# MasterBin-IIAU/Unicorn

Measured on NVIDIA H100. Metric: frames/sec, higher is better.
Workload: dtype bf16

## Files before the change

### include/unicorn_b200.h

```cpp
#ifndef UNICORN_B200_H_
#define UNICORN_B200_H_
#include <stdint.h>

#ifdef __cplusplus
extern "C" {
#endif

#if defined(__GNUC__)
#define UC_API __attribute__((visibility("default")))
#else
#define UC_API
#endif

#define UC_OK 0
#define UC_EINVAL (-1)
#define UC_EDRIVER (-2)
#define UC_ENODEV (-3)

#define UC_BF16 0
#define UC_F32 1
#define UC_F16 2

#define UC_ACT_NONE 0
#define UC_ACT_RELU 1
#define UC_ACT_GELU 2
#define UC_ACT_SILU 3
#define UC_ACT_SIGMOID 4

UC_API const char* uc_last_error(void);
UC_API int uc_version(void);
UC_API int uc_check_device(void);

typedef struct UcConv2d {
  const void* x;
  int x_dtype;
  int B, H, W, Cin, ldx;
  const void* w;
  int Cout, KH, KW, stride, pad;
  const float* bias;
  int act;
  const float* gamma;
  const void* res;
  int ldres;
  void* y;
  int ldy;
  int y_dtype;
  int block_n;
  void* gn_stats;
  int gn_groups;
  const void* row_stats;
  const float* col_s;
  float row_eps;
  int act_after_res;
} UcConv2d;
UC_API int uc_conv2d(const UcConv2d* d, void* stream);

UC_API int uc_stem_ln(const void* img, int img_is_u8_hwc, const float* w48, const float* bias, const float* lnw, const float* lnb,
                      void* out_bf16, int B, int H, int W, int C0, float eps, void* stream);

UC_API int uc_resnet_stem(const void* img, int img_is_u8_hwc, const void* w_f16, const float* bias, void* out_bf16, int B, int H, int W,
                          void* stream);

UC_API int uc_dwconv7_ln(const void* x_bf16, const float* w49, const float* bias, const float* lnw, const float* lnb,
                         void* y_bf16, int B, int H, int W, int C, float eps, void* stream);

UC_API int uc_dwconv7(const void* x_bf16, const float* w49, const float* bias, void* y_bf16, int B, int H, int W, int C,
                      void* ln_stats, int* work_counter, void* stream);

UC_API int uc_dwconv7_mma(const void* x_bf16, const void* qtab, void* y_bf16, int B, int H, int W, int C, int* work_counter, void* stream);

UC_API int uc_convnext_mlp_supported(int C);
UC_API int uc_convnext_mlp(const void* t_bf16, const void* w1f_bf16, const float* c1, const void* w2_bf16, const float* b2, const float* gamma,
                           void* x_bf16, int M, int C, float ln_eps, void* stream);

UC_API int uc_layernorm(const void* x, int ldx, const void* res, int ldres, const float* w, const float* b, void* y,
                        int ldy, long M, int C, float eps, int dtype, void* stream);

UC_API int uc_groupnorm_apply(const void* x, int ldx, const void* stats, const float* w, const float* b, void* y,
                              int ldy, int B, long HW, int C, int G, float eps, int act, const float* prior,
                              const float* beta, const void* add2, int ldadd2, void* y2, int ldy2, void* stream);
UC_API int uc_groupnorm_apply_gather(const void* x, int ldx, int n_src, const void* stats, const float* w, const float* b, void* y,
                                     int ldy, int B, int n_plain, const int* src_of, long HW, int C, int G, float eps, int act,
                                     const float* prior, const float* beta, void* stream);

UC_API int uc_copy_upsample(const void* src, int lds, void* dst, int ldd, int B, int Hs, int Ws, int C, int up, void* stream);
UC_API int uc_pixel_shuffle2(const void* in, int ldi, void* out, int ldo, int B, int H, int W, int Co, void* stream);
UC_API int uc_bilinear_f32(const float* src, float* dst, int P, int Hs, int Ws, int Hd, int Wd, float scale_h,
                           float scale_w, void* stream);
UC_API int uc_letterbox_u8(const uint8_t* src_hwc, int Hs, int Ws, uint8_t* dst_hwc, int Hd, int Wd, int rh, int rw,
                           int swap_rb, int pad, void* stream);
UC_API int uc_letterbox_nv12(const uint8_t* y, const uint8_t* uv, int ld, int Hs, int Ws, uint8_t* dst_hwc, int Hd, int Wd, int rh,
                             int rw, int pad, void* stream);
UC_API int uc_add(const void* a, int lda, const void* b, int ldb, void* y, int ldy, long M, int C, int dtype, void* stream);
UC_API int uc_copy_rows_if(const int* flag_dev, int invert, const void* src, long src_ld_bytes, void* dst, long dst_ld_bytes, long rows,
                           int row_bytes, void* stream);
UC_API int uc_copy_rows_if_batched(const int* flag_dev, const int* gate_dev, int invert, const void* src, long src_ld_bytes, long src_bs_bytes,
                                   void* dst, long dst_ld_bytes, long dst_bs_bytes, long rows, int row_bytes, int B, void* stream);
UC_API int uc_nchw_f32_to_nhwc(const float* src, void* dst, int ldd, int B, int C, long HW, int dtype, void* stream);
UC_API int uc_nhwc_to_nchw_f32(const void* src, int lds, float* dst, int B, int C, long HW, int dtype, void* stream);

UC_API int uc_msda_forward_f32(const float* value, const int64_t* spatial_shapes, const int64_t* level_start_index,
                               const float* sampling_loc, const float* attn_weight, int B, int S, int M, int D, int L,
                               int Lq, int P, float* out, void* stream);
UC_API int uc_msda_fused_bf16(const void* value, const float* offlog, int ld_offlog, void* out, const int* level_hw,
                              int L, int M, int P, void* stream);
UC_API int uc_msda_fused_bf16_batched(const void* value, const float* offlog, int ld_offlog, void* out, const int* level_hw,
                                      int L, int M, int P, int B, void* stream);

UC_API int uc_corr_propagate(const void* embed_ref, int ld_ref, int n_ref, const void* embed_cur, int ld_cur, int n_cur,
                             int C, int dtype, const float* values, int ldv, int n_obj, float* out, int ldo, void* stream);
UC_API int uc_corr_propagate_batched(const void* embed_ref, int ld_ref, long bs_ref, int n_ref, const void* embed_cur, int ld_cur,
                                     long bs_cur, int n_cur, int C, int dtype, const float* values, int ldv, long bs_values, int n_obj,
                                     float* out, int ldo, long bs_out, int B, void* stream);

UC_API int uc_head_decode(const float* const* regobj, const float* const* cls, const int* hw, const int* strides,
                          int ld_ro, int ld_cls, int ncls, float* out, void* stream);
UC_API int uc_head_decode_batched(const float* const* regobj, const float* const* cls, const int* hw, const int* strides,
                                  int ld_ro, int ld_cls, const long* bs_ro, const long* bs_cls, int ncls, int B, float* out,
                                  void* stream);

UC_API long uc_postprocess_workspace_bytes(int max_anchors);
UC_API int uc_postprocess(const float* pred, int A, int ncls, float conf_thre, float nms_thre, int max_keep, void* workspace,
                          long workspace_bytes, float* out_dets, int* out_count, int* out_anchor, void* stream);
UC_API long uc_postprocess_workspace_bytes_batched(int max_anchors, int B);
UC_API int uc_postprocess_batched(const float* pred, int A, int ncls, float conf_thre, float nms_thre, int max_keep, int B,
                                  void* workspace, long workspace_bytes, float* out_dets, int* out_count, int* out_anchor, void* stream);

#define UC_POST_CLASS_AGNOSTIC 1
UC_API int uc_postprocess_batched_ex(const float* pred, int A, int ncls, float conf_thre, float nms_thre, int max_keep, int B, int flags,
                                     void* workspace, long workspace_bytes, float* out_dets, int* out_count, int* out_anchor, void* stream);
UC_API int uc_det_candidates_batched(const float* const* regobj, const float* const* cls, const int* hw, const int* strides, int ld_ro,
                                     int ld_cls, const long* bs_ro, const long* bs_cls, int ncls, int B, float conf_thre, void* workspace,
                                     long workspace_bytes, void* stream);
UC_API int uc_postprocess_nms_batched(int A, float nms_thre, int max_keep, int B, int flags, void* workspace, long workspace_bytes,
                                      float* out_dets, int* out_count, int* out_anchor, void* stream);

UC_API int uc_sample_embed(const void* embed, int ld, int h, int w, int C, int dtype, const float* boxes, int ldb,
                           const int* count_dev, int n_max, float stride, float* out, void* stream);
UC_API int uc_sample_embed_batched(const void* embed, int ld, long bs_embed, int h, int w, int C, int dtype, const float* boxes, int ldb,
                                   long bs_boxes, const int* count_dev, int n_max, float stride, float* out, long bs_out, int B, void* stream);
UC_API int uc_bisoftmax(const float* det_embeds, const float* memo_embeds, int N, int M, int C, const float* det_labels,
                        const float* memo_labels, float* workspace, float* scores, void* stream);
UC_API int uc_qd_assign(const float* scores, int N, int M, const long long* memo_ids, const float* det_scores, int ld_det, float match_thr,
                        float obj_thr, float nms_conf_thr, long long* ids_out, uint8_t* taken_ws, void* stream);
UC_API int uc_box_iou(const float* a, int lda, int N, const float* b, int ldb, int M, float* out, int plus_one, void* stream);

UC_API int uc_aligned_bilinear_add(const void* src, int lds, int hs, int ws, void* dst, int ldd, int C, int factor, void* stream);
UC_API int uc_aligned_bilinear_add_batched(const void* src, int lds, long bs_src, int hs, int ws, void* dst, int ldd, long bs_dst, int C,
                                           int factor, int B, void* stream);
UC_API int uc_dynamic_masks(const float* mask_feats, const float* up_masks, int h, int w, int up_rate, int d_rate,
                            const float* const* dyn_levels, int ld_dyn, const int* level_hw, const int* level_strides,
                            const float* level_soi, const int* anchors_dev, const int* count_dev, int n_max, float* scratch,
                            float* out_masks, void* stream);
UC_API int uc_dynamic_masks_batched(const float* mask_feats, const float* up_masks, int S, int h, int w, int up_rate, int d_rate,
                                    const float* const* dyn_levels, int ld_dyn, const long* bs_dyn, const int* level_hw,
                                    const int* level_strides, const float* level_soi, const int* anchors_dev, long bs_anchors,
                                    const int* count_dev, const int* image_of, int B, int n_max, float* scratch, float* out_masks,
                                    void* stream);

typedef struct UcVosObject {
  const float* mask;
  const uint8_t* init_mask;
  int id;
} UcVosObject;
UC_API int uc_vos_aggregate(const UcVosObject* objs, int n, int Hin, int Win, int H, int W, float r, float* soft_out,
                            uint8_t* seg_out, void* stream);

#define UC_VOS_MAX_VIDEOS UC_MOTS_MAX_IMAGES
typedef struct UcVosVideo {
  const UcVosObject* objs;
  int n;
  int H, W;
  float r;
  float* soft_out;
  uint8_t* seg_out;
} UcVosVideo;
UC_API int uc_vos_aggregate_batched(const UcVosVideo* videos, int B, int Hin, int Win, void* stream);

UC_API long uc_mots_encode_workspace_bytes(int k_max, int H, int W);
UC_API int uc_mots_encode(const float* masks, int n_max, int Hin, int Win, const int* order, const uint8_t* emit, int k, float thr,
                          double r, int H, int W, void* workspace, long workspace_bytes, char* chars, long capacity,
                          long long* offsets, void* stream);

#define UC_MOTS_MAX_IMAGES 64
UC_API int uc_mots_encode_batched(const float* masks, long bs_masks, int n_max, int Hin, int Win, int B, const int* k, const int* H,
                                  const int* W, const double* r, const int* order, const uint8_t* emit, float thr, void* workspace,
                                  long workspace_bytes, char* chars, long capacity, long long* offsets, void* stream);

UC_API int uc_inst_encode_batched(const float* maps, long bs_maps, int n_max, int hs, int ws, int d_rate, int B, const int* count_dev,
                                  int row0, const int* H, const int* W, const double* r, float thr, void* workspace, long workspace_bytes,
                                  uint8_t* emit, char* chars, long capacity, long long* offsets, void* stream);

#define UC_BDD_BAD_CHARS 1
#define UC_BDD_BAD_RUNS 2
#define UC_BDD_BAD_INDEX 4
UC_API long uc_bdd_bitmask_workspace_bytes(int B, const int* k, const int* H, const int* W, long n_chars);
UC_API int uc_bdd_bitmask_batched(int B, const int* k, const int* H, const int* W, const long* out_offsets, const char* chars, long n_chars,
                                  const long long* offsets, const uint32_t* colors, const int* ranks, void* workspace, long workspace_bytes,
                                  uint8_t* out, long out_bytes, int* status, void* stream);

#ifdef __cplusplus
}
#endif
#endif
```

### unicorn_b200/csrc/dwconv_mma.cu

```cuda
#include "uc_ptx.cuh"
#include "uc_common.h"
#include "../../include/unicorn_b200.h"
#include <algorithm>

namespace uc {

constexpr int kMmTW = 16, kMmTH = 16, kMmCH = 32;
constexpr int kMmHW = kMmTW + 8, kMmHH = kMmTH + 6;
constexpr int kMmPixBytes = kMmCH * 2;
constexpr int kMmStageBytes = kMmHH * kMmHW * kMmPixBytes;
constexpr int kMmPlaneBytes = kMmHH * kMmHW * 2;
constexpr int kMmPlanarBytes = kMmCH * kMmPlaneBytes;
constexpr int kMmPairBytes = kMmCH * 7 * 8 * 4;
constexpr int kMmQBytes = kMmPairBytes + kMmCH * 4;
constexpr int kMmSmem = kMmStageBytes + kMmPlanarBytes + kMmQBytes + 128 + 128;
constexpr int kMmWarps = 4, kMmCtasPerSm = 3;

struct alignas(64) DwMmaParams {
  CUtensorMap tmX;
  const uint8_t* qtab;
  uint16_t* y;
  int* work_counter;
  int H, W, C, B, tiles_w, tiles_h, n_items;
};

__device__ __forceinline__ int mm_plane(int c) { return (c & 7) * 4 + (c >> 3); }

__device__ __forceinline__ void bulk_load_1d(void* smem, const void* gmem, uint32_t bytes, uint64_t* bar) {
  asm volatile("cp.async.bulk.shared::cluster.global.mbarrier::complete_tx::bytes [%0], [%1], %2, [%3];" ::"r"(smem_u32(smem)), "l"(gmem),
               "r"(bytes), "r"(smem_u32(bar))
               : "memory");
}

struct DwFrag {
  uint32_t a[2][6];
  uint32_t q[2];
};

__global__ void __launch_bounds__(kMmWarps * 32, kMmCtasPerSm) dwconv7_mma_kernel(const __grid_constant__ DwMmaParams p) {
  constexpr int CPW = kMmCH / kMmWarps;
  extern __shared__ uint8_t dsm_raw[];
  uint8_t* stage = dsm_raw + ((128u - (smem_u32(dsm_raw) & 127u)) & 127u);
  uint8_t* planar = stage + kMmStageBytes;
  uint8_t* qs = planar + kMmPlanarBytes;
  uint64_t* bar = reinterpret_cast<uint64_t*>(qs + kMmQBytes);
  volatile int* s_info = reinterpret_cast<volatile int*>(bar + 2);
  const int lane = threadIdx.x & 31, warp = threadIdx.x >> 5;
  const int g = lane >> 2, t = lane & 3;
  if (threadIdx.x == 0) {
    prefetch_tmap(&p.tmX);
    mbar_init(&bar[0], 1);
    mbar_init(&bar[1], 1);
    fence_barrier_init();
  }
  __syncthreads();
  pdl_wait();
  pdl_launch_dependents();
  const int tiles_img = p.tiles_w * p.tiles_h, tiles_chunk = tiles_img * p.B;
  int static_next = blockIdx.x;
  auto fetch = [&]() {
    if (p.work_counter) return atomicAdd(p.work_counter, 1);
    const int item = static_next;
    static_next += gridDim.x;
    return item;
  };
  auto issue = [&](int slot, int item) {
    volatile int* info = s_info + slot * 4;
    if (item >= p.n_items) {
      info[0] = -1;
      mbar_arrive(&bar[0]);
      return;
    }
    const int chunk = item / tiles_chunk, tt0 = item - chunk * tiles_chunk;
    const int b = tt0 / tiles_img, tt = tt0 - b * tiles_img;
    const int oh0 = (tt / p.tiles_w) * kMmTH, ow0 = (tt % p.tiles_w) * kMmTW;
    info[0] = chunk; info[1] = b; info[2] = oh0; info[3] = ow0;
    mbar_arrive_expect_tx(&bar[0], kMmStageBytes);
    tma_load_4d(stage, &p.tmX, &bar[0], chunk * kMmCH, ow0 - 4, oh0 - 3, b);
  };
  int pending = 0;
  if (threadIdx.x == 0) {
    issue(0, fetch());
    pending = fetch();
  }
  const int fc = warp * CPW;
  const uint32_t planar_w = smem_u32(planar) + mm_plane(fc) * kMmPlaneBytes;
  const uint32_t lm4 = planar_w + static_cast<uint32_t>((((lane & 7) + ((lane >> 3) & 1) * 8) * kMmHW + (lane >> 4) * 8) * 2);
  const uint32_t lm2 = planar_w + static_cast<uint32_t>(((lane & 15) * kMmHW + 16) * 2);
  const int d = 2 * t - g - 1;
  const bool first = d >= -1;
  const uint32_t q_lane = smem_u32(qs) + static_cast<uint32_t>((fc * 7 * 8 + (first ? d + 1 : d + 9)) * 4);
  const float* bias_s = reinterpret_cast<const float*>(qs + kMmPairBytes) + fc;
  const int tq = lane & 3, tsw = (lane >> 2) & 1;
  const uint32_t sel_lo = tsw ? 0x1054u : 0x5410u, sel_hi = tsw ? 0x3276u : 0x7632u;
  auto load_frag = [&](int s, DwFrag& f) {
    const int kh = s % 7;
#pragma unroll
    for (int j = 0; j < 2; ++j) {
      const int c = (s / 7) * 2 + j;
      const uint32_t off = static_cast<uint32_t>(c * 4 * kMmPlaneBytes + kh * (kMmHW * 2));
      asm volatile("ldmatrix.sync.aligned.m8n8.x4.shared.b16 {%0,%1,%2,%3}, [%4];"
                   : "=r"(f.a[j][0]), "=r"(f.a[j][1]), "=r"(f.a[j][2]), "=r"(f.a[j][3]) : "r"(lm4 + off));
      asm volatile("ldmatrix.sync.aligned.m8n8.x2.shared.b16 {%0,%1}, [%2];" : "=r"(f.a[j][4]), "=r"(f.a[j][5]) : "r"(lm2 + off));
      asm volatile("ld.shared.b32 %0, [%1];" : "=r"(f.q[j]) : "r"(q_lane + static_cast<uint32_t>((c * 7 + kh) * 32)));
    }
  };
  int prev_chunk = -1;
  uint32_t q_phase = 0;
  for (int it = 0;; ++it) {
    mbar_wait(&bar[0], it & 1);
    const int chunk = s_info[(it & 1) * 4 + 0];
    if (chunk < 0) break;
    const int b = s_info[(it & 1) * 4 + 1], oh0 = s_info[(it & 1) * 4 + 2], ow0 = s_info[(it & 1) * 4 + 3];
    const int c0 = chunk * kMmCH + fc;
    const bool new_chunk = chunk != prev_chunk;
    prev_chunk = chunk;
    if (new_chunk && threadIdx.x == 0) {
      mbar_arrive_expect_tx(&bar[1], kMmQBytes);
      bulk_load_1d(qs, p.qtab + static_cast<size_t>(chunk) * kMmQBytes, kMmQBytes, &bar[1]);
    }
    {
      const uint4* st = reinterpret_cast<const uint4*>(stage);
#pragma unroll 3
      for (int pp = warp * 8 + (lane >> 2); pp < kMmHH * kMmHW / 2; pp += kMmWarps * 8) {
        const uint4 va = st[(2 * pp + tsw) * 4 + tq];
        const uint4 vb = st[(2 * pp + (tsw ^ 1)) * 4 + tq];
        const uint32_t wa[4] = {va.x, va.y, va.z, va.w}, wb[4] = {vb.x, vb.y, vb.z, vb.w};
        uint8_t* dst = planar + pp * 4;
#pragma unroll
        for (int j = 0; j < 8; ++j)
          *reinterpret_cast<uint32_t*>(dst + mm_plane(tq * 8 + j) * kMmPlaneBytes) = __byte_perm(wa[j >> 1], wb[j >> 1], j & 1 ? sel_hi : sel_lo);
      }
    }
    __syncthreads();
    if (threadIdx.x == 0) {
      issue((it + 1) & 1, pending);
      pending = fetch();
    }
    if (new_chunk) {
      mbar_wait(&bar[1], q_phase);
      q_phase ^= 1;
    }
    if (c0 < p.C) {
      float acc[CPW][2][4];
#pragma unroll
      for (int c = 0; c < CPW; ++c) {
        const float bv = bias_s[c];
#pragma unroll
        for (int e = 0; e < 4; ++e) acc[c][0][e] = acc[c][1][e] = bv;
      }
      DwFrag fr[2];
      load_frag(0, fr[0]);
#pragma unroll
      for (int s = 0; s < CPW / 2 * 7; ++s) {
        if (s + 1 < CPW / 2 * 7) load_frag(s + 1, fr[(s + 1) & 1]);
        const DwFrag& f = fr[s & 1];
#pragma unroll
        for (int j = 0; j < 2; ++j) {
          const int c = (s / 7) * 2 + j;
          const uint32_t b0 = first ? f.q[j] : 0u, b1 = first ? 0u : f.q[j];
#pragma unroll
          for (int nb = 0; nb < 2; ++nb)
            asm volatile("mma.sync.aligned.m16n8k16.row.col.f32.bf16.bf16.f32 {%0,%1,%2,%3}, {%4,%5,%6,%7}, {%8,%9}, {%0,%1,%2,%3};"
                         : "+f"(acc[c][nb][0]), "+f"(acc[c][nb][1]), "+f"(acc[c][nb][2]), "+f"(acc[c][nb][3])
                         : "r"(f.a[j][2 * nb]), "r"(f.a[j][2 * nb + 1]), "r"(f.a[j][2 * nb + 2]), "r"(f.a[j][2 * nb + 3]), "r"(b0), "r"(b1));
        }
      }
      uint16_t* yb = p.y + ((static_cast<size_t>(b) * p.H + oh0) * p.W + ow0) * p.C + c0;
#pragma unroll
      for (int nb = 0; nb < 2; ++nb)
#pragma unroll
        for (int e = 0; e < 4; ++e) {
          const int r = g + (e >> 1) * 8, cl = nb * 8 + 2 * t + (e & 1);
          if (oh0 + r < p.H && ow0 + cl < p.W) {
            uint4 o;
            o.x = pack_bf16(acc[0][nb][e], acc[1][nb][e]); o.y = pack_bf16(acc[2][nb][e], acc[3][nb][e]);
            o.z = pack_bf16(acc[4][nb][e], acc[5][nb][e]); o.w = pack_bf16(acc[6][nb][e], acc[7][nb][e]);
            *reinterpret_cast<uint4*>(yb + (static_cast<size_t>(r) * p.W + cl) * p.C) = o;
          }
        }
    }
    __syncthreads();
  }
}

}

using namespace uc;

extern "C" int uc_dwconv7_mma(const void* x_bf16, const void* qtab, void* y_bf16, int B, int H, int W, int C,
                              int* work_counter, void* stream_v) {
  cudaStream_t stream = static_cast<cudaStream_t>(stream_v);
  if (!x_bf16 || !qtab || !y_bf16) return set_error(UC_EINVAL, "uc_dwconv7_mma: null pointer");
  if (x_bf16 == y_bf16) return set_error(UC_EINVAL, "uc_dwconv7_mma: not an in-place operation");
  if (B < 1 || H < 1 || W < 1 || C < 8 || C % 8) return set_error(UC_EINVAL, "uc_dwconv7_mma: C must be a multiple of 8");
  if ((reinterpret_cast<uintptr_t>(x_bf16) | reinterpret_cast<uintptr_t>(y_bf16) | reinterpret_cast<uintptr_t>(qtab)) & 15) return set_error(UC_EINVAL, "uc_dwconv7_mma: 16-byte aligned maps");
  int rc = ensure_driver();
  if (rc) return rc;
  DwMmaParams p;
  memset(&p, 0, sizeof(p));
  {
    uint64_t dims[4] = {static_cast<uint64_t>(C), static_cast<uint64_t>(W), static_cast<uint64_t>(H), static_cast<uint64_t>(B)};
    uint64_t strides[3] = {static_cast<uint64_t>(C) * 2, static_cast<uint64_t>(W) * C * 2, static_cast<uint64_t>(H) * W * C * 2};
    uint32_t box[4] = {kMmCH, kMmHW, kMmHH, 1};
    rc = encode_tmap(&p.tmX, CU_TENSOR_MAP_DATA_TYPE_BFLOAT16, 4, x_bf16, dims, strides, box, CU_TENSOR_MAP_SWIZZLE_NONE);
    if (rc) return rc;
  }
  p.qtab = static_cast<const uint8_t*>(qtab);
  p.y = static_cast<uint16_t*>(y_bf16);
  p.work_counter = work_counter;
  p.H = H; p.W = W; p.C = C; p.B = B;
  p.tiles_w = (W + kMmTW - 1) / kMmTW;
  p.tiles_h = (H + kMmTH - 1) / kMmTH;
  const long items = static_cast<long>(p.tiles_w) * p.tiles_h * B * ((C + kMmCH - 1) / kMmCH);
  if (items > 0x7fffffffL) return set_error(UC_EINVAL, "uc_dwconv7_mma: too many tiles");
  p.n_items = static_cast<int>(items);
  static PerDeviceFlag attr_dev;
  bool& attr = attr_dev.get();
  if (!attr) {
    cudaError_t e = cudaFuncSetAttribute(dwconv7_mma_kernel, cudaFuncAttributeMaxDynamicSharedMemorySize, kMmSmem);
    if (e != cudaSuccess) return set_error(static_cast<int>(e), "uc_dwconv7_mma: cudaFuncSetAttribute: %s", cudaGetErrorString(e));
    attr = true;
  }
  const int grid = static_cast<int>(std::min<long>(items, static_cast<long>(num_sms()) * kMmCtasPerSm));
  cudaError_t e = launch_pdl(dwconv7_mma_kernel, dim3(grid), dim3(kMmWarps * 32), kMmSmem, stream, p);
  if (e != cudaSuccess) return set_error(static_cast<int>(e), "uc_dwconv7_mma launch: %s", cudaGetErrorString(e));
  return check_launch("uc_dwconv7_mma");
}
```

### unicorn_b200/ops.py

```python
import ctypes

import torch

from . import _lib
from ._lib import BF16, F32, F16, ACT_NONE, ACT_RELU, ACT_GELU, ACT_SILU, ACT_SIGMOID

_DT = {torch.bfloat16: BF16, torch.float32: F32, torch.float16: F16}


def _p(t):
    return ctypes.c_void_p(t.data_ptr()) if t is not None else None


def _nhwc_ld(t):
    assert t.dim() == 4 and t.is_cuda, "expected a CUDA NHWC tensor"
    B, H, W, C = t.shape
    ld = t.stride(2) if W > 1 else (t.stride(1) // W if H > 1 else max(C, t.stride(2)))
    assert t.stride(3) == 1 or C == 1
    if W > 1:
        assert t.stride(2) == ld
    if H > 1:
        assert t.stride(1) == W * ld, (t.shape, t.stride())
    if B > 1:
        assert t.stride(0) == H * W * ld
    return ld


def pack_conv_weight(w, dtype=torch.bfloat16, cout_pad=8):
    if w.dim() == 2:
        w = w[:, :, None, None]
    Cout, Cin, KH, KW = w.shape
    Cp = (Cout + cout_pad - 1) // cout_pad * cout_pad
    out = torch.zeros(Cp, KH * KW, Cin, dtype=dtype, device=w.device)
    out[:Cout] = w.permute(0, 2, 3, 1).reshape(Cout, KH * KW, Cin).to(dtype)
    return out.contiguous()


CONV_TRACE = None


def conv2d(x, w_packed, KH, KW, stride=1, pad=0, bias=None, act=ACT_NONE, gamma=None, res=None, out=None,
           out_dtype=None, block_n=0, gn_stats=None, gn_groups=0, row_stats=None, col_s=None, row_eps=1e-6, act_after_res=False):
    B, H, W, Cin = x.shape
    Cout = w_packed.shape[0]
    assert w_packed.shape[1] == KH * KW and w_packed.shape[2] == Cin and w_packed.is_contiguous()
    assert w_packed.dtype == x.dtype
    Ho = (H + 2 * pad - KH) // stride + 1
    Wo = (W + 2 * pad - KW) // stride + 1
    if out is None:
        out = torch.empty(B, Ho, Wo, Cout, dtype=out_dtype or x.dtype, device=x.device)
    assert out.shape == (B, Ho, Wo, Cout), (out.shape, (B, Ho, Wo, Cout))
    d = _lib.UcConv2d()
    d.x, d.x_dtype = _p(x), _DT[x.dtype]
    d.B, d.H, d.W, d.Cin, d.ldx = B, H, W, Cin, _nhwc_ld(x)
    d.w = _p(w_packed)
    d.Cout, d.KH, d.KW, d.stride, d.pad = Cout, KH, KW, stride, pad
    d.bias, d.act, d.gamma = _p(bias), act, _p(gamma)
    if bias is not None:
        assert bias.dtype == torch.float32 and bias.numel() >= Cout
    if gamma is not None:
        assert gamma.dtype == torch.float32 and gamma.numel() >= Cout
    d.res, d.ldres = _p(res), (_nhwc_ld(res) if res is not None else 0)
    if res is not None:
        assert res.dtype == out.dtype and res.shape == out.shape
    d.y, d.ldy, d.y_dtype = _p(out), _nhwc_ld(out), _DT[out.dtype]
    d.block_n = block_n
    d.gn_stats, d.gn_groups = _p(gn_stats), gn_groups
    d.row_stats, d.col_s, d.row_eps = _p(row_stats), _p(col_s), row_eps
    d.act_after_res = int(bool(act_after_res))
    if row_stats is not None:
        assert row_stats.dtype == torch.int64 and row_stats.numel() == B * H * W * 2 and col_s is not None and col_s.numel() >= Cout
    if CONV_TRACE is not None:
        CONV_TRACE.append(dict(M=B * Ho * Wo, N=Cout, K=Cin * KH * KW, k=KH, s=stride, bn=block_n, act=act, gn=gn_groups,
                               f32=int(out.dtype == torch.float32)))
    _lib.check(_lib.lib().uc_conv2d(ctypes.byref(d), _lib.stream_ptr()), "uc_conv2d")
    return out


def linear(x2d, w_packed, **kw):
    M, K = x2d.shape
    assert x2d.stride(1) == 1
    x4 = x2d.as_strided((1, 1, M, K), (M * x2d.stride(0), M * x2d.stride(0), x2d.stride(0), 1))
    out = kw.pop("out", None)
    res = kw.pop("res", None)
    if out is not None:
        out = out.as_strided((1, 1, M, out.shape[1]), (M * out.stride(0), M * out.stride(0), out.stride(0), 1))
    if res is not None:
        res = res.as_strided((1, 1, M, res.shape[1]), (M * res.stride(0), M * res.stride(0), res.stride(0), 1))
    y = conv2d(x4, w_packed, 1, 1, out=out, res=res, **kw)
    return y.as_strided((M, y.shape[3]), (y.stride(2), 1))


def _L():
    return _lib.lib()


def _S():
    return _lib.stream_ptr()


_f = ctypes.c_float
_i = ctypes.c_int
_l = ctypes.c_long


def pack_stem_weight(w):
    return w.reshape(w.shape[0], 48).t().contiguous().float()


def pack_dw_weight(w):
    return w.reshape(w.shape[0], 49).t().contiguous().float()


def pack_dw_weight_mma(w, bias):
    C = w.shape[0]
    Cp = -(-C // 32) * 32
    e = torch.zeros(Cp, 7, 9, dtype=torch.bfloat16, device=w.device)
    e[:C, :, 1:8] = w.reshape(C, 7, 7).to(torch.bfloat16)
    bits = e.view(torch.int16).to(torch.int32) & 0xffff
    pairs = (bits[:, :, 0:8] | (bits[:, :, 1:9] << 16)).to(torch.int32).reshape(Cp // 32, 32 * 7 * 8)
    bp = torch.zeros(Cp, dtype=torch.float32, device=w.device)
    bp[:C] = bias.float()
    return torch.cat([pairs, bp.view(torch.int32).reshape(Cp // 32, 32)], dim=1).contiguous()


def dwconv7_mma(x, qtab, out=None, work_counter=None):
    B, H, W, C = x.shape
    assert x.is_contiguous() and x.dtype == torch.bfloat16 and qtab.dtype == torch.int32 and qtab.shape == (-(-C // 32), 1824)
    if out is None:
        out = torch.empty_like(x)
    _lib.check(_L().uc_dwconv7_mma(_p(x), _p(qtab), _p(out), B, H, W, C, _p(work_counter), _S()), "uc_dwconv7_mma")
    return out


def convnext_mlp_supported(C):
    return bool(_L().uc_convnext_mlp_supported(int(C)))


def convnext_mlp(t, w1f, c1, w2, b2, gamma, x, eps=1e-6):
    M, C = t.shape
    assert t.is_contiguous() and x.is_contiguous() and x.shape == t.shape and t.dtype == x.dtype == torch.bfloat16
    assert w1f.dtype == torch.bfloat16 and w1f.numel() == 4 * C * C and w2.dtype == torch.bfloat16 and w2.numel() == 4 * C * C
    _lib.check(_L().uc_convnext_mlp(_p(t), _p(w1f), _p(c1), _p(w2), _p(b2), _p(gamma), _p(x), M, C, ctypes.c_float(eps), _S()), "uc_convnext_mlp")
    return x


def stem_ln(img, w48, bias, lnw, lnb, eps=1e-6):
    u8 = img.dtype == torch.uint8
    if u8:
        B, H, W, _ = img.shape
    else:
        B, _, H, W = img.shape
        assert img.dtype == torch.float32
    assert img.is_contiguous()
    C0 = w48.shape[1]
    out = torch.empty(B, H // 4, W // 4, C0, dtype=torch.bfloat16, device=img.device)
    _lib.check(_L().uc_stem_ln(_p(img), int(u8), _p(w48), _p(bias), _p(lnw), _p(lnb), _p(out), B, H, W, C0, _f(eps), _S()), "uc_stem_ln")
    return out


def pack_resnet_stem_weight(w):
    out = torch.zeros(w.shape[0], 160, dtype=torch.float16, device=w.device)
    out[:, :147] = w.reshape(w.shape[0], 147).to(torch.float16)
    return out


def resnet_stem(img, w160, bias, out=None):
    u8 = img.dtype == torch.uint8
    if u8:
        B, H, W, _ = img.shape
    else:
        B, _, H, W = img.shape
        assert img.dtype == torch.float32
    assert img.is_contiguous() and w160.dtype == torch.float16 and w160.shape == (64, 160) and bias.dtype == torch.float32
    if out is None:
        out = torch.empty(B, H // 4, W // 4, 64, dtype=torch.bfloat16, device=img.device)
    assert out.shape == (B, H // 4, W // 4, 64) and out.is_contiguous() and out.dtype == torch.bfloat16
    _lib.check(_L().uc_resnet_stem(_p(img), int(u8), _p(w160), _p(bias), _p(out), B, H, W, _S()), "uc_resnet_stem")
    return out


def dwconv7_ln(x, w49, bias, lnw, lnb, eps=1e-6, out=None):
    B, H, W, C = x.shape
    assert x.is_contiguous() and x.dtype == torch.bfloat16
    if out is None:
        out = torch.empty_like(x)
    _lib.check(_L().uc_dwconv7_ln(_p(x), _p(w49), _p(bias), _p(lnw), _p(lnb), _p(out), B, H, W, C, _f(eps), _S()), "uc_dwconv7_ln")
    return out


def dwconv7(x, w49, bias, out=None, ln_stats=None, work_counter=None):
    B, H, W, C = x.shape
    assert x.is_contiguous() and x.dtype == torch.bfloat16
    if out is None:
        out = torch.empty_like(x)
    if ln_stats is not None:
        assert ln_stats.dtype == torch.int64 and ln_stats.is_contiguous() and ln_stats.numel() == B * H * W * 2
    if work_counter is not None:
        assert work_counter.dtype == torch.int32 and work_counter.numel() >= 1
    _lib.check(_L().uc_dwconv7(_p(x), _p(w49), _p(bias), _p(out), B, H, W, C, _p(ln_stats), _p(work_counter), _S()), "uc_dwconv7")
    return out


def layernorm(x2d, w, b, eps, res=None, out=None):
    M, C = x2d.shape
    if out is None:
        out = torch.empty(M, C, dtype=x2d.dtype, device=x2d.device)
    _lib.check(_L().uc_layernorm(_p(x2d), x2d.stride(0), _p(res), res.stride(0) if res is not None else 0, _p(w), _p(b),
                                 _p(out), out.stride(0), _l(M), C, _f(eps), _DT[x2d.dtype], _S()), "uc_layernorm")
    return out


def groupnorm_apply(x, stats, w, b, G, eps, act, out=None, prior=None, beta=None, add2=None, out2=None):
    B, H, W, C = x.shape
    if out is None:
        out = x
    ld2 = _nhwc_ld(add2) if add2 is not None else 0
    _lib.check(_L().uc_groupnorm_apply(_p(x), _nhwc_ld(x), _p(stats), _p(w), _p(b), _p(out), _nhwc_ld(out), B, _l(H * W), C, G,
                                       _f(eps), act, _p(prior), _p(beta), _p(add2), ld2, _p(out2),
                                       _nhwc_ld(out2) if out2 is not None else 0, _S()), "uc_groupnorm_apply")
    return out


def copy_upsample(src, dst, up):
    B, Hs, Ws, C = src.shape
    assert dst.shape == (B, Hs * up, Ws * up, C)
    _lib.check(_L().uc_copy_upsample(_p(src), _nhwc_ld(src), _p(dst), _nhwc_ld(dst), B, Hs, Ws, C, up, _S()), "uc_copy_upsample")
    return dst


def pixel_shuffle2(x, out=None):
    B, H, W, C4 = x.shape
    Co = C4 // 4
    if out is None:
        out = torch.empty(B, 2 * H, 2 * W, Co, dtype=x.dtype, device=x.device)
    _lib.check(_L().uc_pixel_shuffle2(_p(x), _nhwc_ld(x), _p(out), _nhwc_ld(out), B, H, W, Co, _S()), "uc_pixel_shuffle2")
    return out


def bilinear(src, Hd, Wd, scale_h=0.0, scale_w=0.0, out=None):
    Hs, Ws = src.shape[-2:]
    P = src.numel() // (Hs * Ws)
    if out is None:
        out = torch.empty(*src.shape[:-2], Hd, Wd, dtype=torch.float32, device=src.device)
    _lib.check(_L().uc_bilinear_f32(_p(src), _p(out), P, Hs, Ws, Hd, Wd, _f(scale_h), _f(scale_w), _S()), "uc_bilinear_f32")
    return out


def add(a2d, b2d, out=None):
    M, C = a2d.shape
    if out is None:
        out = torch.empty(M, C, dtype=a2d.dtype, device=a2d.device)
    _lib.check(_L().uc_add(_p(a2d), a2d.stride(0), _p(b2d), b2d.stride(0), _p(out), out.stride(0), _l(M), C, _DT[a2d.dtype], _S()), "uc_add")
    return out


def copy_rows_if(flag, src, dst, invert=False, gate=None):
    assert src.shape == dst.shape and src.dtype == dst.dtype and flag.dtype == torch.int32
    B, C = src.shape[0], src.shape[-1]
    es = src.element_size()
    if B == 1 and gate is None:
        rows = src.numel() // C
        _lib.check(_L().uc_copy_rows_if(_p(flag), int(bool(invert)), _p(src), _l(_nhwc_ld(src) * es), _p(dst), _l(_nhwc_ld(dst) * es), _l(rows), C * es, _S()),
                   "uc_copy_rows_if")
        return dst
    assert src.dim() == 4 and flag.numel() == B and (gate is None or (gate.dtype == torch.int32 and gate.numel() == B))
    rows = src.numel() // (B * C)
    lds, ldd = _nhwc_ld(src), _nhwc_ld(dst)
    _lib.check(_L().uc_copy_rows_if_batched(_p(flag), _p(gate), int(bool(invert)), _p(src), _l(lds * es), _l(rows * lds * es), _p(dst), _l(ldd * es),
                                            _l(rows * ldd * es), _l(rows), C * es, B, _S()), "uc_copy_rows_if_batched")
    return dst


def letterbox_u8(src, input_size, swap_rb=True, pad=114, out=None):
    assert src.dtype == torch.uint8 and src.is_cuda and src.is_contiguous() and src.dim() == 3 and src.shape[2] == 3
    h, w = src.shape[:2]
    H, W = input_size
    r = min(H / h, W / w)
    if out is None:
        out = torch.empty(1, H, W, 3, dtype=torch.uint8, device=src.device)
    _lib.check(_L().uc_letterbox_u8(_p(src), h, w, _p(out), H, W, int(h * r), int(w * r), int(bool(swap_rb)), int(pad), _S()), "uc_letterbox_u8")
    return out, r


def nchw_to_nhwc(x, dtype=torch.bfloat16, out=None):
    B, C, H, W = x.shape
    assert x.dtype == torch.float32 and x.is_contiguous()
    if out is None:
        out = torch.empty(B, H, W, C, dtype=dtype, device=x.device)
    _lib.check(_L().uc_nchw_f32_to_nhwc(_p(x), _p(out), _nhwc_ld(out), B, C, _l(H * W), _DT[out.dtype], _S()), "uc_nchw_f32_to_nhwc")
    return out


def nhwc_to_nchw(x):
    B, H, W, C = x.shape
    assert x.dtype in (torch.bfloat16, torch.float16), "uc_nhwc_to_nchw_f32 converts 16-bit NHWC maps"
    out = torch.empty(B, C, H, W, dtype=torch.float32, device=x.device)
    _lib.check(_L().uc_nhwc_to_nchw_f32(_p(x), _nhwc_ld(x), _p(out), B, C, _l(H * W), _DT[x.dtype], _S()), "uc_nhwc_to_nchw_f32")
    return out


def msda_forward(value, spatial_shapes, level_start_index, sampling_loc, attn_weight):
    B, S, M, D = value.shape
    _, Lq, _, L, P, _ = sampling_loc.shape
    out = torch.empty(B, Lq, M * D, dtype=torch.float32, device=value.device)
    _lib.check(_L().uc_msda_forward_f32(_p(value), _p(spatial_shapes), _p(level_start_index), _p(sampling_loc), _p(attn_weight),
                                        B, S, M, D, L, Lq, P, _p(out), _S()), "uc_msda_forward_f32")
    return out


def msda_fused(value, offlog, level_hw, M=8, P=4, out=None):
    L = len(level_hw)
    Lq = sum(h * w for h, w in level_hw)
    B = value.shape[0] // Lq
    assert value.shape == (B * Lq, M * 32) and B >= 1 and value.dtype == torch.bfloat16 and value.is_contiguous()
    assert offlog.dtype == torch.float32 and offlog.shape[0] == B * Lq and offlog.shape[1] >= M * L * P * 3
    if out is None:
        out = torch.empty(B * Lq, M * 32, dtype=torch.bfloat16, device=value.device)
    hw = (ctypes.c_int * (2 * L))(*[v for pair in level_hw for v in pair])
    if B == 1:
        _lib.check(_L().uc_msda_fused_bf16(_p(value), _p(offlog), offlog.stride(0), _p(out), hw, L, M, P, _S()), "uc_msda_fused_bf16")
    else:
        _lib.check(_L().uc_msda_fused_bf16_batched(_p(value), _p(offlog), offlog.stride(0), _p(out), hw, L, M, P, B, _S()),
                   "uc_msda_fused_bf16_batched")
    return out


def corr_propagate(embed_ref, embed_cur, values, out=None):
    if embed_ref.dim() == 2:
        n_ref, C = embed_ref.shape
        n_cur = embed_cur.shape[0]
        n_obj = values.shape[0]
        assert values.dtype == torch.float32 and values.stride(1) == 1 and values.shape[1] == n_ref
        if out is None:
            out = torch.empty(n_obj, n_cur, dtype=torch.float32, device=values.device)
        _lib.check(_L().uc_corr_propagate(_p(embed_ref), embed_ref.stride(0), n_ref, _p(embed_cur), embed_cur.stride(0), n_cur, C,
                                          _DT[embed_ref.dtype], _p(values), values.stride(0), n_obj, _p(out), out.stride(0), _S()),
                   "uc_corr_propagate")
        return out
    B, n_ref, C = embed_ref.shape
    n_cur = embed_cur.shape[1]
    n_obj = values.shape[1]
    assert embed_cur.shape[0] == B and values.shape[0] == B and values.shape[2] == n_ref
    assert values.dtype == torch.float32 and values.stride(2) == 1 and embed_ref.stride(2) == 1 and embed_cur.stride(2) == 1
    if out is None:
        out = torch.empty(B, n_obj, n_cur, dtype=torch.float32, device=values.device)
    assert out.shape == (B, n_obj, n_cur) and out.stride(2) == 1
    _lib.check(_L().uc_corr_propagate_batched(_p(embed_ref), embed_ref.stride(1), _l(embed_ref.stride(0)), n_ref, _p(embed_cur),
                                              embed_cur.stride(1), _l(embed_cur.stride(0)), n_cur, C, _DT[embed_ref.dtype], _p(values),
                                              values.stride(1), _l(values.stride(0)), n_obj, _p(out), out.stride(1), _l(out.stride(0)), B,
                                              _S()), "uc_corr_propagate_batched")
    return out


def head_decode(regobj, cls, hw, strides, ncls, out=None):
    A = sum(h * w for h, w in hw)
    B = regobj[0].shape[0] if regobj[0].dim() == 4 else 1
    if out is None:
        out = torch.empty(B, A, 5 + ncls, dtype=torch.float32, device=regobj[0].device)
    ro = (ctypes.c_void_p * 3)(*[t.data_ptr() for t in regobj])
    cl = (ctypes.c_void_p * 3)(*[t.data_ptr() for t in cls])
    hwa = (ctypes.c_int * 6)(*[v for pair in hw for v in pair])
    st = (ctypes.c_int * 3)(*strides)
    if B == 1:
        _lib.check(_L().uc_head_decode(ro, cl, hwa, st, regobj[0].shape[-1], cls[0].shape[-1], ncls, _p(out), _S()), "uc_head_decode")
        return out
    assert all(t.dim() == 4 and t.shape[0] == B for t in list(regobj) + list(cls)) and out.shape == (B, A, 5 + ncls) and out.is_contiguous()
    bs_ro = (ctypes.c_long * 3)(*[t.stride(0) for t in regobj])
    bs_cl = (ctypes.c_long * 3)(*[t.stride(0) for t in cls])
    _lib.check(_L().uc_head_decode_batched(ro, cl, hwa, st, regobj[0].shape[-1], cls[0].shape[-1], bs_ro, bs_cl, ncls, B, _p(out), _S()),
               "uc_head_decode_batched")
    return out


class PostWorkspace:

    def __init__(self, max_anchors, device, batch=1):
        fn = _L().uc_postprocess_workspace_bytes_batched
        fn.restype = ctypes.c_long
        self.nbytes = fn(max_anchors, batch)
        assert self.nbytes > 0, "PostWorkspace: batch must be >= 1"
        lead = (batch,) if batch > 1 else ()
        self.buf = torch.empty(self.nbytes, dtype=torch.uint8, device=device)
        self.dets = torch.empty(*lead, max_anchors, 7, dtype=torch.float32, device=device)
        self.count = torch.zeros(batch, dtype=torch.int32, device=device)
        self.anchors = torch.zeros(*lead, max_anchors, dtype=torch.int32, device=device)
        self.max_anchors, self.batch = max_anchors, batch


def postprocess_device(pred, ncls, conf, nms, ws, max_keep=0):
    assert pred.is_contiguous() and pred.dtype == torch.float32 and pred.shape[-2] <= ws.max_anchors
    if pred.dim() == 3 and pred.shape[0] == 1:
        pred = pred[0]
    if pred.dim() == 2:
        A = pred.shape[0]
        _lib.check(_L().uc_postprocess(_p(pred), A, ncls, _f(conf), _f(nms), int(max_keep), _p(ws.buf), _l(ws.nbytes), _p(ws.dets), _p(ws.count), _p(ws.anchors), _S()),
                   "uc_postprocess", 4)
        return ws.dets, ws.count
    B, A = pred.shape[:2]
    assert B == ws.batch and A == ws.max_anchors, "postprocess_device: a batch of B images needs a PostWorkspace(A, device, batch=B)"
    _lib.check(_L().uc_postprocess_batched(_p(pred), A, ncls, _f(conf), _f(nms), int(max_keep), B, _p(ws.buf), _l(ws.nbytes), _p(ws.dets),
                                           _p(ws.count), _p(ws.anchors), _S()), "uc_postprocess_batched", 4)
    return ws.dets, ws.count


def sample_embed(embed, boxes, n_max, stride=8.0, count=None, out=None):
    B, h, w, C = embed.shape
    if boxes.dim() == 2:
        if out is None:
            out = torch.zeros(n_max, C, dtype=torch.float32, device=embed.device)
        _lib.check(_L().uc_sample_embed(_p(embed), _nhwc_ld(embed), h, w, C, _DT[embed.dtype], _p(boxes), boxes.stride(0), _p(count), n_max,
                                        _f(stride), _p(out), _S()), "uc_sample_embed")
        return out
    assert boxes.shape[0] == B and boxes.shape[1] >= n_max and boxes.stride(2) == 1 and count is not None and count.numel() == B
    if out is None:
        out = torch.zeros(B, n_max, C, dtype=torch.float32, device=embed.device)
    assert out.shape == (B, n_max, C) and out.dtype == torch.float32 and out.stride(2) == 1 and out.stride(1) == C
    if B == 1:
        _lib.check(_L().uc_sample_embed(_p(embed), _nhwc_ld(embed), h, w, C, _DT[embed.dtype], _p(boxes), boxes.stride(1), _p(count), n_max,
                                        _f(stride), _p(out), _S()), "uc_sample_embed")
        return out
    _lib.check(_L().uc_sample_embed_batched(_p(embed), _nhwc_ld(embed), _l(embed.stride(0)), h, w, C, _DT[embed.dtype], _p(boxes), boxes.stride(1),
                                            _l(boxes.stride(0)), _p(count), n_max, _f(stride), _p(out), _l(out.stride(0)), B, _S()),
               "uc_sample_embed_batched")
    return out


def bisoftmax(det_embeds, memo_embeds, det_labels=None, memo_labels=None):
    N, C = det_embeds.shape
    M = memo_embeds.shape[0]
    ws = torch.empty(N * M + 2 * N + 2 * M, dtype=torch.float32, device=det_embeds.device)
    scores = torch.empty(N, M, dtype=torch.float32, device=det_embeds.device)
    _lib.check(_L().uc_bisoftmax(_p(det_embeds), _p(memo_embeds), N, M, C, _p(det_labels), _p(memo_labels), _p(ws), _p(scores), _S()),
               "uc_bisoftmax", 3)
    return scores
# ... 118 lines not shown
```

Measured before the change: 183.5.

## Add 16-channel dwconv7 MMA variant chosen automatically for small grids

```diff
diff --git a/include/unicorn_b200.h b/include/unicorn_b200.h
--- a/include/unicorn_b200.h
+++ b/include/unicorn_b200.h
@@ -69,6 +69,11 @@
 
 UC_API int uc_dwconv7_mma(const void* x_bf16, const void* qtab, void* y_bf16, int B, int H, int W, int C, int* work_counter, void* stream);
 
+UC_API int uc_dwconv7_mma_geom(const void* x_bf16, const void* qtab, void* y_bf16, int B, int H, int W, int C, int* work_counter,
+                               int chans_per_item, void* stream);
+
+UC_API int uc_dwconv7_mma_plan(int B, int H, int W, int C, int sms, int chans_per_item, int* out);
+
 UC_API int uc_convnext_mlp_supported(int C);
 UC_API int uc_convnext_mlp(const void* t_bf16, const void* w1f_bf16, const float* c1, const void* w2_bf16, const float* b2, const float* gamma,
                            void* x_bf16, int M, int C, float ln_eps, void* stream);
diff --git a/unicorn_b200/csrc/dwconv_mma.cu b/unicorn_b200/csrc/dwconv_mma.cu
--- a/unicorn_b200/csrc/dwconv_mma.cu
+++ b/unicorn_b200/csrc/dwconv_mma.cu
@@ -5,16 +5,29 @@
 
 namespace uc {
 
-constexpr int kMmTW = 16, kMmTH = 16, kMmCH = 32;
+constexpr int kMmTW = 16, kMmTH = 16;
 constexpr int kMmHW = kMmTW + 8, kMmHH = kMmTH + 6;
-constexpr int kMmPixBytes = kMmCH * 2;
-constexpr int kMmStageBytes = kMmHH * kMmHW * kMmPixBytes;
 constexpr int kMmPlaneBytes = kMmHH * kMmHW * 2;
-constexpr int kMmPlanarBytes = kMmCH * kMmPlaneBytes;
-constexpr int kMmPairBytes = kMmCH * 7 * 8 * 4;
-constexpr int kMmQBytes = kMmPairBytes + kMmCH * 4;
-constexpr int kMmSmem = kMmStageBytes + kMmPlanarBytes + kMmQBytes + 128 + 128;
-constexpr int kMmWarps = 4, kMmCtasPerSm = 3;
+constexpr int kMmQChunkBytes = 32 * 7 * 8 * 4 + 32 * 4;
+constexpr int kMmSmemPerSm = 233472, kMmCtaReserved = 1024;
+constexpr int kMmWarpsPerSm = 12;
+
+template <int NW>
+struct DwMma {
+  static constexpr int CH = 8 * NW;
+  static constexpr int StageBytes = kMmHH * kMmHW * CH * 2;
+  static constexpr int PlanarBytes = CH * kMmPlaneBytes;
+  static constexpr int PairBytes = CH * 7 * 8 * 4;
+  static constexpr int QBytes = PairBytes + CH * 4;
+  static constexpr int Smem = StageBytes + PlanarBytes + QBytes + 128 + 128;
+  static constexpr int CtasPerSm = std::min(kMmWarpsPerSm / NW, kMmSmemPerSm / (Smem + kMmCtaReserved));
+  static __host__ __device__ constexpr int plane(int c) {
+    return NW == 4 ? (c & 7) * 4 + (c >> 3) : ((c & 7) >> 1) * 4 + (c & 1) + 2 * (c >> 3);
+  }
+};
+static_assert(DwMma<4>::Smem == 75136 && DwMma<4>::CtasPerSm == 3, "NW = 4 is the 32-channel item of 3 CTAs per SM");
+static_assert(DwMma<2>::CtasPerSm == 6, "6 CTAs per SM of the 16-channel item");
+static_assert(DwMma<4>::Smem <= 232448, "227 KB per CTA");
 
 struct alignas(64) DwMmaParams {
   CUtensorMap tmX;
@@ -24,8 +37,6 @@
   int H, W, C, B, tiles_w, tiles_h, n_items;
 };
 
-__device__ __forceinline__ int mm_plane(int c) { return (c & 7) * 4 + (c >> 3); }
-
 __device__ __forceinline__ void bulk_load_1d(void* smem, const void* gmem, uint32_t bytes, uint64_t* bar) {
   asm volatile("cp.async.bulk.shared::cluster.global.mbarrier::complete_tx::bytes [%0], [%1], %2, [%3];" ::"r"(smem_u32(smem)), "l"(gmem),
                "r"(bytes), "r"(smem_u32(bar))
@@ -37,13 +48,16 @@
   uint32_t q[2];
 };
 
-__global__ void __launch_bounds__(kMmWarps * 32, kMmCtasPerSm) dwconv7_mma_kernel(const __grid_constant__ DwMmaParams p) {
-  constexpr int CPW = kMmCH / kMmWarps;
+template <int NW>
+__global__ void __launch_bounds__(NW * 32, kMmWarpsPerSm / NW) dwconv7_mma_kernel(const __grid_constant__ DwMmaParams p) {
+  using G = DwMma<NW>;
+  constexpr int CH = G::CH;
+  constexpr int CPW = 8;
   extern __shared__ uint8_t dsm_raw[];
   uint8_t* stage = dsm_raw + ((128u - (smem_u32(dsm_raw) & 127u)) & 127u);
-  uint8_t* planar = stage + kMmStageBytes;
-  uint8_t* qs = planar + kMmPlanarBytes;
-  uint64_t* bar = reinterpret_cast<uint64_t*>(qs + kMmQBytes);
+  uint8_t* planar = stage + G::StageBytes;
+  uint8_t* qs = planar + G::PlanarBytes;
+  uint64_t* bar = reinterpret_cast<uint64_t*>(qs + G::QBytes);
   volatile int* s_info = reinterpret_cast<volatile int*>(bar + 2);
   const int lane = threadIdx.x & 31, warp = threadIdx.x >> 5;
   const int g = lane >> 2, t = lane & 3;
@@ -75,8 +89,8 @@
     const int b = tt0 / tiles_img, tt = tt0 - b * tiles_img;
     const int oh0 = (tt / p.tiles_w) * kMmTH, ow0 = (tt % p.tiles_w) * kMmTW;
     info[0] = chunk; info[1] = b; info[2] = oh0; info[3] = ow0;
-    mbar_arrive_expect_tx(&bar[0], kMmStageBytes);
-    tma_load_4d(stage, &p.tmX, &bar[0], chunk * kMmCH, ow0 - 4, oh0 - 3, b);
+    mbar_arrive_expect_tx(&bar[0], G::StageBytes);
+    tma_load_4d(stage, &p.tmX, &bar[0], chunk * CH, ow0 - 4, oh0 - 3, b);
   };
   int pending = 0;
   if (threadIdx.x == 0) {
@@ -84,21 +98,21 @@
     pending = fetch();
   }
   const int fc = warp * CPW;
-  const uint32_t planar_w = smem_u32(planar) + mm_plane(fc) * kMmPlaneBytes;
+  const uint32_t planar_w = smem_u32(planar) + G::plane(fc) * kMmPlaneBytes;
   const uint32_t lm4 = planar_w + static_cast<uint32_t>((((lane & 7) + ((lane >> 3) & 1) * 8) * kMmHW + (lane >> 4) * 8) * 2);
   const uint32_t lm2 = planar_w + static_cast<uint32_t>(((lane & 15) * kMmHW + 16) * 2);
   const int d = 2 * t - g - 1;
   const bool first = d >= -1;
   const uint32_t q_lane = smem_u32(qs) + static_cast<uint32_t>((fc * 7 * 8 + (first ? d + 1 : d + 9)) * 4);
-  const float* bias_s = reinterpret_cast<const float*>(qs + kMmPairBytes) + fc;
-  const int tq = lane & 3, tsw = (lane >> 2) & 1;
+  const float* bias_s = reinterpret_cast<const float*>(qs + G::PairBytes) + fc;
+  const int tq = lane % NW, ti = lane / NW, tsw = (ti * NW / 4) & 1;
   const uint32_t sel_lo = tsw ? 0x1054u : 0x5410u, sel_hi = tsw ? 0x3276u : 0x7632u;
   auto load_frag = [&](int s, DwFrag& f) {
     const int kh = s % 7;
 #pragma unroll
     for (int j = 0; j < 2; ++j) {
       const int c = (s / 7) * 2 + j;
-      const uint32_t off = static_cast<uint32_t>(c * 4 * kMmPlaneBytes + kh * (kMmHW * 2));
+      const uint32_t off = static_cast<uint32_t>((G::plane(c) - G::plane(0)) * kMmPlaneBytes + kh * (kMmHW * 2));
       asm volatile("ldmatrix.sync.aligned.m8n8.x4.shared.b16 {%0,%1,%2,%3}, [%4];"
                    : "=r"(f.a[j][0]), "=r"(f.a[j][1]), "=r"(f.a[j][2]), "=r"(f.a[j][3]) : "r"(lm4 + off));
       asm volatile("ldmatrix.sync.aligned.m8n8.x2.shared.b16 {%0,%1}, [%2];" : "=r"(f.a[j][4]), "=r"(f.a[j][5]) : "r"(lm2 + off));
@@ -112,24 +126,27 @@
     const int chunk = s_info[(it & 1) * 4 + 0];
     if (chunk < 0) break;
     const int b = s_info[(it & 1) * 4 + 1], oh0 = s_info[(it & 1) * 4 + 2], ow0 = s_info[(it & 1) * 4 + 3];
-    const int c0 = chunk * kMmCH + fc;
+    const int c0 = chunk * CH + fc;
     const bool new_chunk = chunk != prev_chunk;
     prev_chunk = chunk;
     if (new_chunk && threadIdx.x == 0) {
-      mbar_arrive_expect_tx(&bar[1], kMmQBytes);
-      bulk_load_1d(qs, p.qtab + static_cast<size_t>(chunk) * kMmQBytes, kMmQBytes, &bar[1]);
+      const int q32 = chunk * CH / 32, sub = chunk * CH % 32;
+      const uint8_t* src = p.qtab + static_cast<size_t>(q32) * kMmQChunkBytes;
+      mbar_arrive_expect_tx(&bar[1], G::QBytes);
+      bulk_load_1d(qs, src + sub * (7 * 8 * 4), G::PairBytes, &bar[1]);
+      bulk_load_1d(qs + G::PairBytes, src + 32 * 7 * 8 * 4 + sub * 4, CH * 4, &bar[1]);
     }
     {
       const uint4* st = reinterpret_cast<const uint4*>(stage);
 #pragma unroll 3
-      for (int pp = warp * 8 + (lane >> 2); pp < kMmHH * kMmHW / 2; pp += kMmWarps * 8) {
-        const uint4 va = st[(2 * pp + tsw) * 4 + tq];
-        const uint4 vb = st[(2 * pp + (tsw ^ 1)) * 4 + tq];
+      for (int pp = warp * (32 / NW) + ti; pp < kMmHH * kMmHW / 2; pp += 32) {
+        const uint4 va = st[(2 * pp + tsw) * NW + tq];
+        const uint4 vb = st[(2 * pp + (tsw ^ 1)) * NW + tq];
         const uint32_t wa[4] = {va.x, va.y, va.z, va.w}, wb[4] = {vb.x, vb.y, vb.z, vb.w};
         uint8_t* dst = planar + pp * 4;
 #pragma unroll
         for (int j = 0; j < 8; ++j)
-          *reinterpret_cast<uint32_t*>(dst + mm_plane(tq * 8 + j) * kMmPlaneBytes) = __byte_perm(wa[j >> 1], wb[j >> 1], j & 1 ? sel_hi : sel_lo);
+          *reinterpret_cast<uint32_t*>(dst + G::plane(tq * 8 + j) * kMmPlaneBytes) = __byte_perm(wa[j >> 1], wb[j >> 1], j & 1 ? sel_hi : sel_lo);
       }
     }
     __syncthreads();
@@ -184,25 +201,65 @@
   }
 }
 
-}
-
-using namespace uc;
-
-extern "C" int uc_dwconv7_mma(const void* x_bf16, const void* qtab, void* y_bf16, int B, int H, int W, int C,
-                              int* work_counter, void* stream_v) {
+struct DwPlan {
+  int nw, items, ctas_per_sm, grid, smem;
+};
+
+int dw_items(int B, int H, int W, int C, int nw) {
+  const long items = static_cast<long>((W + kMmTW - 1) / kMmTW) * ((H + kMmTH - 1) / kMmTH) * B * ((C + 8 * nw - 1) / (8 * nw));
+  return items > 0x7fffffffL ? -1 : static_cast<int>(items);
+}
+
+int dw_ctas_per_sm(int nw) { return nw == 4 ? DwMma<4>::CtasPerSm : DwMma<2>::CtasPerSm; }
+int dw_smem(int nw) { return nw == 4 ? DwMma<4>::Smem : DwMma<2>::Smem; }
+
+int dw_choose_nw(int B, int H, int W, int C, int sms) {
+  return 2L * dw_items(B, H, W, C, 4) <= static_cast<long>(sms) * DwMma<4>::CtasPerSm ? 2 : 4;
+}
+
+DwPlan dw_plan(int B, int H, int W, int C, int sms, int nw) {
+  if (nw == 0) nw = dw_choose_nw(B, H, W, C, sms);
+  DwPlan pl;
+  pl.nw = nw;
+  pl.items = dw_items(B, H, W, C, nw);
+  pl.ctas_per_sm = dw_ctas_per_sm(nw);
+  pl.grid = static_cast<int>(std::min<long>(pl.items, static_cast<long>(sms) * pl.ctas_per_sm));
+  pl.smem = dw_smem(nw);
+  return pl;
+}
+
+template <int NW>
+int dw_launch(const DwMmaParams& p, int grid, cudaStream_t stream) {
+  static PerDeviceFlag attr_dev;
+  bool& attr = attr_dev.get();
+  if (!attr) {
+    cudaError_t e = cudaFuncSetAttribute(dwconv7_mma_kernel<NW>, cudaFuncAttributeMaxDynamicSharedMemorySize, DwMma<NW>::Smem);
+    if (e != cudaSuccess) return set_error(static_cast<int>(e), "uc_dwconv7_mma: cudaFuncSetAttribute: %s", cudaGetErrorString(e));
+    attr = true;
+  }
+  cudaError_t e = launch_pdl(dwconv7_mma_kernel<NW>, dim3(grid), dim3(NW * 32), DwMma<NW>::Smem, stream, p);
+  if (e != cudaSuccess) return set_error(static_cast<int>(e), "uc_dwconv7_mma launch: %s", cudaGetErrorString(e));
+  return 0;
+}
+
+int dwconv7_mma_run(const void* x_bf16, const void* qtab, void* y_bf16, int B, int H, int W, int C, int* work_counter, int nw,
+                    void* stream_v) {
   cudaStream_t stream = static_cast<cudaStream_t>(stream_v);
   if (!x_bf16 || !qtab || !y_bf16) return set_error(UC_EINVAL, "uc_dwconv7_mma: null pointer");
   if (x_bf16 == y_bf16) return set_error(UC_EINVAL, "uc_dwconv7_mma: not an in-place operation");
   if (B < 1 || H < 1 || W < 1 || C < 8 || C % 8) return set_error(UC_EINVAL, "uc_dwconv7_mma: C must be a multiple of 8");
   if ((reinterpret_cast<uintptr_t>(x_bf16) | reinterpret_cast<uintptr_t>(y_bf16) | reinterpret_cast<uintptr_t>(qtab)) & 15) return set_error(UC_EINVAL, "uc_dwconv7_mma: 16-byte aligned maps");
+  if (nw != 0 && nw != 2 && nw != 4) return set_error(UC_EINVAL, "uc_dwconv7_mma: channels per item must be 16 or 32");
+  if (dw_items(B, H, W, C, nw ? nw : 2) < 0) return set_error(UC_EINVAL, "uc_dwconv7_mma: too many tiles");
   int rc = ensure_driver();
   if (rc) return rc;
+  const DwPlan pl = dw_plan(B, H, W, C, num_sms(), nw);
   DwMmaParams p;
   memset(&p, 0, sizeof(p));
   {
     uint64_t dims[4] = {static_cast<uint64_t>(C), static_cast<uint64_t>(W), static_cast<uint64_t>(H), static_cast<uint64_t>(B)};
     uint64_t strides[3] = {static_cast<uint64_t>(C) * 2, static_cast<uint64_t>(W) * C * 2, static_cast<uint64_t>(H) * W * C * 2};
-    uint32_t box[4] = {kMmCH, kMmHW, kMmHH, 1};
+    uint32_t box[4] = {static_cast<uint32_t>(8 * pl.nw), kMmHW, kMmHH, 1};
     rc = encode_tmap(&p.tmX, CU_TENSOR_MAP_DATA_TYPE_BFLOAT16, 4, x_bf16, dims, strides, box, CU_TENSOR_MAP_SWIZZLE_NONE);
     if (rc) return rc;
   }
@@ -212,18 +269,35 @@
   p.H = H; p.W = W; p.C = C; p.B = B;
   p.tiles_w = (W + kMmTW - 1) / kMmTW;
   p.tiles_h = (H + kMmTH - 1) / kMmTH;
-  const long items = static_cast<long>(p.tiles_w) * p.tiles_h * B * ((C + kMmCH - 1) / kMmCH);
-  if (items > 0x7fffffffL) return set_error(UC_EINVAL, "uc_dwconv7_mma: too many tiles");
-  p.n_items = static_cast<int>(items);
-  static PerDeviceFlag attr_dev;
-  bool& attr = attr_dev.get();
-  if (!attr) {
-    cudaError_t e = cudaFuncSetAttribute(dwconv7_mma_kernel, cudaFuncAttributeMaxDynamicSharedMemorySize, kMmSmem);
-    if (e != cudaSuccess) return set_error(static_cast<int>(e), "uc_dwconv7_mma: cudaFuncSetAttribute: %s", cudaGetErrorString(e));
-    attr = true;
-  }
-  const int grid = static_cast<int>(std::min<long>(items, static_cast<long>(num_sms()) * kMmCtasPerSm));
-  cudaError_t e = launch_pdl(dwconv7_mma_kernel, dim3(grid), dim3(kMmWarps * 32), kMmSmem, stream, p);
-  if (e != cudaSuccess) return set_error(static_cast<int>(e), "uc_dwconv7_mma launch: %s", cudaGetErrorString(e));
+  p.n_items = pl.items;
+  rc = pl.nw == 4 ? dw_launch<4>(p, pl.grid, stream) : dw_launch<2>(p, pl.grid, stream);
+  if (rc) return rc;
   return check_launch("uc_dwconv7_mma");
 }
+
+}
+
+using namespace uc;
+
+extern "C" int uc_dwconv7_mma(const void* x_bf16, const void* qtab, void* y_bf16, int B, int H, int W, int C,
+                              int* work_counter, void* stream_v) {
+  return dwconv7_mma_run(x_bf16, qtab, y_bf16, B, H, W, C, work_counter, 0, stream_v);
+}
+
+extern "C" int uc_dwconv7_mma_geom(const void* x_bf16, const void* qtab, void* y_bf16, int B, int H, int W, int C,
+                                   int* work_counter, int chans_per_item, void* stream_v) {
+  if (chans_per_item != 0 && chans_per_item != 16 && chans_per_item != 32)
+    return set_error(UC_EINVAL, "uc_dwconv7_mma: channels per item must be 16 or 32");
+  return dwconv7_mma_run(x_bf16, qtab, y_bf16, B, H, W, C, work_counter, chans_per_item / 8, stream_v);
+}
+
+extern "C" int uc_dwconv7_mma_plan(int B, int H, int W, int C, int sms, int chans_per_item, int* out) {
+  if (!out || B < 1 || H < 1 || W < 1 || C < 8 || C % 8 || sms < 1) return set_error(UC_EINVAL, "uc_dwconv7_mma_plan: bad shape");
+  if (chans_per_item != 0 && chans_per_item != 16 && chans_per_item != 32)
+    return set_error(UC_EINVAL, "uc_dwconv7_mma_plan: channels per item must be 16 or 32");
+  if (dw_items(B, H, W, C, 2) < 0) return set_error(UC_EINVAL, "uc_dwconv7_mma_plan: too many tiles");
+  const DwPlan pl = dw_plan(B, H, W, C, sms, chans_per_item / 8);
+  const int o[] = {8 * pl.nw, kMmTH, kMmTW, pl.ctas_per_sm, pl.grid, pl.smem, 8 * pl.nw, kMmHW, kMmHH, pl.items};
+  memcpy(out, o, sizeof(o));
+  return 0;
+}
diff --git a/unicorn_b200/ops.py b/unicorn_b200/ops.py
--- a/unicorn_b200/ops.py
+++ b/unicorn_b200/ops.py
@@ -124,13 +124,27 @@
     return torch.cat([pairs, bp.view(torch.int32).reshape(Cp // 32, 32)], dim=1).contiguous()
 
 
-def dwconv7_mma(x, qtab, out=None, work_counter=None):
+def dwconv7_mma(x, qtab, out=None, work_counter=None, chans_per_item=None):
     B, H, W, C = x.shape
     assert x.is_contiguous() and x.dtype == torch.bfloat16 and qtab.dtype == torch.int32 and qtab.shape == (-(-C // 32), 1824)
     if out is None:
         out = torch.empty_like(x)
-    _lib.check(_L().uc_dwconv7_mma(_p(x), _p(qtab), _p(out), B, H, W, C, _p(work_counter), _S()), "uc_dwconv7_mma")
-    return out
+    if chans_per_item is None:
+        rc = _L().uc_dwconv7_mma(_p(x), _p(qtab), _p(out), B, H, W, C, _p(work_counter), _S())
+    else:
+        rc = _L().uc_dwconv7_mma_geom(_p(x), _p(qtab), _p(out), B, H, W, C, _p(work_counter), chans_per_item, _S())
+    _lib.check(rc, "uc_dwconv7_mma")
+    return out
+
+
+DW_PLAN_FIELDS = ("chans_per_item", "tile_h", "tile_w", "ctas_per_sm", "grid", "smem_bytes", "box_c", "box_w", "box_h", "items")
+
+
+def dwconv7_mma_plan(B, H, W, C, sms, chans_per_item=0):
+    out = (ctypes.c_int * len(DW_PLAN_FIELDS))()
+    if _L().uc_dwconv7_mma_plan(B, H, W, C, sms, chans_per_item, out) != 0:
+        raise _lib.UnicornB200Error("uc_dwconv7_mma_plan: " + _L().uc_last_error().decode("utf-8", "replace"))
+    return dict(zip(DW_PLAN_FIELDS, out))
 
 
 def convnext_mlp_supported(C):
```

New measurement: 184.1, median of 6. No clear change (+0.3%).
